# pfac-lib/PFAC

Hardware: AMD Instinct MI355X
Metric: input GB/s scanned (PFAC_matchFromDevice, bit-exact) (higher is better)
Workload: dtype u8

## Files before the change

### pfac_amd/csrc/scan_filter.hip

```cpp
#include "scan_common.h"

namespace {


#ifndef PFAC_ABLATE
#define PFAC_ABLATE 0
#endif
#ifndef PFAC_STATS
#define PFAC_STATS 0
#endif
constexpr int kGroupTiles = pfac::kChunkTiles;
constexpr int kGroupBytes = kGroupTiles * kTileBytes;
constexpr int kStageWords = (kGroupBytes + 48) / 4;
#ifndef PFAC_REFILL_MIN
#define PFAC_REFILL_MIN 16
#endif
#ifndef PFAC_REFILL_BATCH
#define PFAC_REFILL_BATCH 1
#endif
#ifndef PFAC_TIMING
#define PFAC_TIMING 0
#endif
#ifndef PFAC_LIST_CAP
#define PFAC_LIST_CAP 128
#endif
constexpr uint32_t kListCap = PFAC_LIST_CAP;
#ifndef PFAC_REDUCE_PARTS
#define PFAC_REDUCE_PARTS 32
#endif
#ifndef PFAC_APPEND_MIN
#define PFAC_APPEND_MIN 48
#endif
constexpr uint32_t kAppendMin = PFAC_APPEND_MIN;
#ifndef PFAC_MERGE_MIN
#define PFAC_MERGE_MIN 48
#endif
constexpr uint32_t kMergeMin = PFAC_MERGE_MIN;
static_assert(kMergeMin <= 64 && kMergeMin < kListCap, "left-over candidates are moved to the list's head one per lane");
#ifndef PFAC_PATCH_STAGED
#define PFAC_PATCH_STAGED 0
#endif
constexpr bool kStagedPatch = PFAC_PATCH_STAGED != 0;
constexpr uint32_t kReduceCap = 16;
#ifndef PFAC_FRONT_LOG2
#define PFAC_FRONT_LOG2 4
#endif

#ifndef PFAC_WRITERS
#define PFAC_WRITERS 3
#endif
#ifndef PFAC_SPAN_LOG2
#define PFAC_SPAN_LOG2 2
#endif
constexpr int kSpanLog2 = PFAC_SPAN_LOG2;
constexpr uint32_t kSpanChunks = 1u << kSpanLog2;
#ifndef PFAC_RUN_AHEAD
#define PFAC_RUN_AHEAD ((64u >> kSpanLog2) > 4u ? (64u >> kSpanLog2) : 4u)
#endif
constexpr uint32_t kRunAhead = PFAC_RUN_AHEAD;
constexpr uint32_t kRing = 2 * kRunAhead;
static_assert((kRing - kRunAhead) * kSpanChunks >= 2 * 16 + kSpanChunks, "ring slack covers the unresolved tickets of 16 waves");
constexpr uint32_t kEnd = 0xFFFFFFFFu;
struct Control {
    uint32_t popCount;
    uint32_t pubCount;
    uint32_t claimTurn;
    uint32_t endSpan;
    uint32_t ring[kRing];
};
constexpr int kControlWords = (sizeof(Control) / 4 + 3) / 4 * 4;

template <bool REDUCE, bool STAGE, int VETO = 0>
struct FilterLds {
    static constexpr bool kStageWalk = !REDUCE && STAGE;
    static constexpr int kWriters = REDUCE ? 0 : PFAC_WRITERS;
    static constexpr int kScanners = kWavesPerBlock - kWriters;
    static constexpr int kStageBufWords = kStageWalk ? (int)(kWalkStageBytes / 4) : kStageWords;
    static constexpr int kStageBufs = kStageWalk ? 2 : 1;
    enum Region { kQueue, kQueueB, kQueueC, kStage, kList, kPairs, kDense, kTrailing };
    static constexpr uint32_t kWaveWords[kTrailing] = {
        kQueueCap * (kStageWalk ? 1 : 4),
        kStageWalk ? 0 : kQueueCap * 2,
        (REDUCE || kStageWalk) ? 0 : kQueueCap * 4,
        (uint32_t)(kStageBufWords * kStageBufs),
        kListCap / 2,
        (REDUCE || kStagedPatch) ? 2 * kReduceCap : 0,
        REDUCE ? 0 : kDenseStage,
    };
    static constexpr uint32_t offsetWords(int r)
    {
        uint32_t w = kControlWords;
        for (int i = 0; i < r; i++) w += kScanners * kWaveWords[i];
        return w;
    }
    template <int R> static constexpr uint32_t kOffsetWords = offsetWords(R);
    static constexpr size_t kBufferBytes = 4 * (size_t)offsetWords(kTrailing);
    static constexpr size_t bytes(int log2BitsLad, int log2BitsF3, bool hasShort)
    {
        return (REDUCE ? pfac::reduceBitmapLdsBytes(log2BitsF3, hasShort) : pfac::filterBitmapLdsBytes(log2BitsLad, log2BitsF3, hasShort)) + kBufferBytes;
    }
};

__device__ __forceinline__ uint32_t ldsLoad(const uint32_t *p) { return __hip_atomic_load(p, __ATOMIC_RELAXED, __HIP_MEMORY_SCOPE_WORKGROUP); }
__device__ __forceinline__ void ldsStore(uint32_t *p, uint32_t v) { __hip_atomic_store(p, v, __ATOMIC_RELAXED, __HIP_MEMORY_SCOPE_WORKGROUP); }


__device__ __forceinline__ uint32_t waveMin(uint32_t v)
{
    auto step = [](uint32_t x, uint32_t y) { return y < x ? y : x; };
    v = step(v, (uint32_t)__builtin_amdgcn_update_dpp((int)v, (int)v, 0x111, 0xf, 0xf, false));
    v = step(v, (uint32_t)__builtin_amdgcn_update_dpp((int)v, (int)v, 0x112, 0xf, 0xf, false));
    v = step(v, (uint32_t)__builtin_amdgcn_update_dpp((int)v, (int)v, 0x114, 0xf, 0xf, false));
    v = step(v, (uint32_t)__builtin_amdgcn_update_dpp((int)v, (int)v, 0x118, 0xf, 0xf, false));
    v = step(v, (uint32_t)__builtin_amdgcn_update_dpp((int)v, (int)v, 0x142, 0xa, 0xf, false));
    v = step(v, (uint32_t)__builtin_amdgcn_update_dpp((int)v, (int)v, 0x143, 0xc, 0xf, false));
    return (uint32_t)__builtin_amdgcn_readlane((int)v, 63);
}

#ifndef PFAC_COMPILER_VGPRS
#define PFAC_COMPILER_VGPRS 59
#endif
constexpr int kCompilerVgprs = PFAC_COMPILER_VGPRS;

template <bool TEX, bool HAS_SHORT, bool REDUCE, int kWalkSets, bool STAGE, int VETO = 0>
__global__ __launch_bounds__(kBlockThreads, PFAC_MIN_WAVES_PER_SIMD) __attribute__((amdgpu_num_vgpr(kCompilerVgprs)))
void pfac_scan_filter(ScanArgs a)
{
    constexpr int kTilesPerIter = kGroupTiles;
    constexpr int kChunkBytes = kTilesPerIter * kTileBytes;
    using WCtx = ChainCtx<TEX>;
    constexpr uint32_t kEntry = (REDUCE || (!STAGE && VETO == 2)) ? kEntryBytes : kEntryBytesFull;
    constexpr bool kWideEntry = kEntry > kEntryBytes;
    using L = FilterLds<REDUCE, STAGE, VETO>;
    constexpr bool kStageWalk = L::kStageWalk;
    constexpr bool kVeto = !REDUCE && !STAGE && VETO != 0;
    constexpr bool kVetoG = kVeto && VETO == 2;
    constexpr uint32_t kListCapK = kVetoG ? 2u * kListCap : kListCap;
    static_assert(kListCapK * 2 <= kQueueCap * 16 || !kVetoG, "VETO = 2: the list lies in the place of the queue's bytes 20..35");
#ifndef PFAC_TAIL_ASK_MIN
#define PFAC_TAIL_ASK_MIN 8
#endif
    constexpr uint32_t kTailAskMin = PFAC_TAIL_ASK_MIN;
    using WLane = std::conditional_t<kStageWalk, StageLane<TEX>, ChainLane<TEX, kEntry, kVeto && VETO == 1>>;
    constexpr int kStageWordsK = L::kStageBufWords, kStageBufs = L::kStageBufs;
    constexpr int kHaloDwords = kStageWalk ? (int)(kWalkHalo / 4) : 12;
    extern __shared__ __attribute__((aligned(16))) unsigned char smem[];
    const int words3 = 1 << (a.log2Bits - 5), wordsLad = 1 << (a.log2BitsLad - 5), wordsF3 = 1 << (a.log2BitsF3 - 5);
    uint32_t *sGram3 = reinterpret_cast<uint32_t *>(smem);
    uint32_t *sLadder = sGram3 + kLadderLdsOffset / 4;
    uint32_t *sFinal3 = REDUCE ? sGram3 + (kGram1LdsOffset + kGram1LdsBytes) / 4 : sLadder + wordsLad;
    uint32_t *sShort = sFinal3 + wordsF3;
    constexpr int kWriters = L::kWriters, kScanners = L::kScanners;
    constexpr uint32_t kQCap = kQueueCap;
    Control *ctl = reinterpret_cast<Control *>(sShort + (HAS_SHORT ? pfac::kShortLdsBytes / 4 : 0));
    uint32_t *const sBuffers = reinterpret_cast<uint32_t *>(ctl);
    uint32_t *sQueueAll = sBuffers + L::template kOffsetWords<L::kQueue>;
    uint32_t *sQueueBAll = sBuffers + L::template kOffsetWords<L::kQueueB>, *sQueueCAll = sBuffers + L::template kOffsetWords<L::kQueueC>;
    uint32_t *sStageAll = sBuffers + L::template kOffsetWords<L::kStage>, *sListAll = sBuffers + L::template kOffsetWords<L::kList>;
    uint32_t *sReduceAll = sBuffers + L::template kOffsetWords<L::kPairs>, *sDenseAll = sBuffers + L::template kOffsetWords<L::kDense>;
    uint32_t *sHotAll = sBuffers + L::template kOffsetWords<L::kTrailing>;

    const int tid = threadIdx.x;
    if (__builtin_amdgcn_groupstaticsize() != 0) __builtin_trap();
    {
        auto copy16 = [&](uint32_t *dst, const void *src, int words) {
            const u32x4 *g = reinterpret_cast<const u32x4 *>(src);
            u32x4 *s = reinterpret_cast<u32x4 *>(dst);
            for (int i = tid; i < words / 4; i += kBlockThreads) s[i] = g[i];
        };
        if (REDUCE) {
            copy16(sGram3, a.prefix4, (int)(kPrefix4LdsBytes / 4));
            copy16(sGram3 + kGram1LdsOffset / 4, a.gram1, (int)(kGram1LdsBytes / 4));
        } else {
            copy16(sGram3, a.gram3, words3);
            copy16(sLadder, a.ladder, wordsLad);
        }
        copy16(sFinal3, a.final3, wordsF3);
        if (HAS_SHORT) copy16(sShort, a.shortBits, (int)(pfac::kShortLdsBytes / 4));
        if constexpr (kStageWalk) copy16(sHotAll, a.chainSlots, (int)a.hotSlots * 4);
        if constexpr (kVeto && !kVetoG) { if (a.tail != nullptr) copy16(sHotAll, a.tail, 3 << a.log2Tail); }
        if (tid < kControlWords) reinterpret_cast<uint32_t *>(ctl)[tid] = (tid == (int)(offsetof(Control, endSpan) / 4)) ? kEnd : 0u;
    }
    __syncthreads();

    const int lane = tid & 63;
    const int wave = __builtin_amdgcn_readfirstlane(tid >> 6);
    u32x4 *queue = reinterpret_cast<u32x4 *>(sQueueAll) + wave * kQCap;
    typedef uint32_t u32x2 __attribute__((ext_vector_type(2)));
    u32x2 *queueB = reinterpret_cast<u32x2 *>(sQueueBAll) + wave * kQCap;
    u32x4 *queueC = reinterpret_cast<u32x4 *>(sQueueCAll) + wave * kQCap;
    uint32_t *const stage0 = sStageAll + wave * (kStageWordsK * kStageBufs);
    uint32_t *stage = stage0;
    uint32_t *queue32 = sQueueAll + wave * kQCap;
    StageView view;
    view.addr[0] = (uint32_t)(reinterpret_cast<unsigned char *>(stage0) - smem);
    view.addr[1] = view.addr[0] + (uint32_t)kStageWordsK * 4u;
    view.base[0] = view.base[1] = 0;
    uint32_t cur = 0, qEnd[2] = {0, 0};
    bool modeStage = kStageWalk && __builtin_amdgcn_readfirstlane((int)a.work[pfac::kModeHintWord]) != 0;
    uint32_t deepRecent = 0, stageHold = modeStage ? 8u : 0u;
    uint16_t *list = kVetoG ? reinterpret_cast<uint16_t *>(sQueueCAll + wave * kQCap * 4) : reinterpret_cast<uint16_t *>(sListAll + wave * (kListCap / 2));
    const uint32_t n = (uint32_t)a.n;
    const Lds lds{sGram3, sLadder, sFinal3, sShort,
                  ((1u << ((uint32_t)a.log2Bits - 5u)) - 1u) << 2 , 32u - (uint32_t)a.log2BitsLad, 32u - (uint32_t)a.log2BitsF3};
#if PFAC_LADDER_BLOCKED
    uint32_t vLadMask;
    asm volatile("v_mov_b32 %0, %1" : "=v"(vLadMask) : "s"(((1u << ((uint32_t)a.log2BitsLad - 5u)) - 1u) << 2));
    auto ladWord = [&](uint32_t h) -> uint32_t {
        uint32_t addr;
        asm("v_and_b32_sdwa %0, %1, %2 dst_sel:DWORD dst_unused:UNUSED_PAD src0_sel:WORD_1 src1_sel:DWORD" : "=v"(addr) : "v"(h), "v"(vLadMask));
        return *reinterpret_cast<const __attribute__((address_space(3))) uint32_t *>(addr + kLadderLdsOffset);
    };
    auto ladStop = [](uint32_t w, uint32_t h) -> uint32_t { return (w >> ((h >> 3) & 31u)) & (w >> ((h >> 8) & 31u)); };
    auto ladGoOn = [](uint32_t w, uint32_t h) -> uint32_t { return w >> ((h >> 13) & 31u); };
    auto ladGoOn2 = [](uint32_t w, uint32_t h) -> uint32_t { return w >> (h & 31u); };
#else
    auto ladProbe = [&](uint32_t v) -> uint32_t {
        const uint32_t idx = v >> lds.shiftLad;
        return *reinterpret_cast<const __attribute__((address_space(3))) uint32_t *>(((idx >> 3) & ~3u) + kLadderLdsOffset) >> (idx & 31u);
    };
    auto ladWord = [](uint32_t h) -> uint32_t { return h; };
    auto ladStop = [&](uint32_t, uint32_t h) -> uint32_t { return ladProbe(h) & ladProbe(h * pfac::kLadMulS); };
    auto ladGoOn = [&](uint32_t, uint32_t h) -> uint32_t { return ladProbe(h * pfac::kLadMulG); };
    auto ladGoOn2 = [&](uint32_t, uint32_t h) -> uint32_t { return ladProbe(h * pfac::kLadMulG2); };
#endif
    WCtx wctx(a);
    if constexpr (kStageWalk) {
        wctx.hotAddr = (uint32_t)(reinterpret_cast<unsigned char *>(sHotAll) - smem);
        wctx.hotSlots = a.hotSlots;
    }
    WLane walk[kWalkSets];
    bool alive[kWalkSets];
#pragma unroll
    for (int s = 0; s < kWalkSets; s++) alive[s] = false;
    uint32_t qh = 0, qv = 0;
    constexpr uint32_t kMask = kQCap - 1;
    auto uni = [](uint32_t v) { return (uint32_t)__builtin_amdgcn_readfirstlane((int)v); };
    uint32_t stRounds = 0, stLaneSteps = 0, stStarts = 0, stHits = 0, stCand = 0;
#if PFAC_STATS
    uint32_t stFullRounds = 0, stSlotGathers = 0, stWinLoads = 0, stStartDead = 0;
#endif

    uint32_t *rPos = sReduceAll + wave * (2 * kReduceCap);
    uint32_t *rId = rPos + kReduceCap;
    uint32_t rn = 0;
    int pendMatch[kWalkSets];
    uint32_t pendPos[kWalkSets];
#pragma unroll
    for (int s = 0; s < kWalkSets; s++) { pendMatch[s] = 0; pendPos[s] = 0; }

    auto report = [&](bool ended, const WLane &w, int s) {
        if (ended & (w.match != 0)) {
            if (REDUCE || kStagedPatch) {
                pendMatch[s] = w.match;
                pendPos[s] = w.pos;
            } else {
#if defined(PFAC_EXP_PATCH_LOCAL)
                a.out[w.pos & 0xFFFFFu] = w.match;
#elif defined(PFAC_EXP_PATCH_NT)
                __builtin_nontemporal_store(w.match, &a.out[w.pos]);
#elif !defined(PFAC_EXP_NOSTORE)
                a.out[w.pos] = w.match;
#endif
            }
        }
    };
    auto flushStaged = [&]() {
        if (rn == 0) return;
        __builtin_amdgcn_fence(__ATOMIC_RELEASE, "wavefront");
        __builtin_amdgcn_fence(__ATOMIC_ACQUIRE, "wavefront");
        if (REDUCE) {
            unsigned int base = 0;
            if (lane == 0) base = atomicAdd(a.reduceCount, rn);
            base = (unsigned int)__builtin_amdgcn_readfirstlane((int)base);
            for (uint32_t i = lane; i < rn; i += 64) {
                a.out[base + i] = (int)rId[i];
                a.reducePos[base + i] = (int)(a.reduceBase + rPos[i]);
            }
        } else {
            if ((uint32_t)lane < rn) a.out[rPos[lane]] = (int)rId[lane];
        }
        rn = 0;
        __builtin_amdgcn_fence(__ATOMIC_RELEASE, "wavefront");
    };
    auto stagePending = [&]() {
        if (!REDUCE && !kStagedPatch) return;
#pragma unroll
        for (int s = 0; s < kWalkSets; s++) {
            const bool has = pendMatch[s] != 0;
            const uint64_t m = __ballot(has);
            if (m) {
                const uint32_t cnt = (uint32_t)__popcll(m);
                if (rn + cnt > kReduceCap) flushStaged();
                if (cnt > kReduceCap) {
                    if (REDUCE) {
                        unsigned int base = 0;
                        if (lane == 0) base = atomicAdd(a.reduceCount, cnt);
                        base = (unsigned int)__builtin_amdgcn_readfirstlane((int)base) + laneRankIn(m);
                        if (has) { a.out[base] = pendMatch[s]; a.reducePos[base] = (int)(a.reduceBase + pendPos[s]); pendMatch[s] = 0; }
                    } else if (has) {
                        a.out[pendPos[s]] = pendMatch[s];
                        pendMatch[s] = 0;
                    }
                } else {
                    const uint32_t at = rn + laneRankIn(m);
                    if (has) { rPos[at] = pendPos[s]; rId[at] = (uint32_t)pendMatch[s]; pendMatch[s] = 0; }
                    rn = uni(rn + cnt);
                }
            }
        }
    };
    constexpr bool kSpecKernel = WLane::kSpec;
    constexpr uint32_t kSpecOnScore = 16, kSpecOffRounds = 16;
#ifndef PFAC_SPEC_FORCE
#define PFAC_SPEC_FORCE -1
#endif
    int advBalance = 0;
    uint32_t chunkEvents = 0;
    bool specOn = PFAC_SPEC_FORCE == 1 || (PFAC_SPEC_FORCE < 0 && kStageWalk && modeStage);
    uint32_t specScore = 0, specIdle = 0;
    auto walkIssue = [&]() {
#pragma unroll
        for (int s = 0; s < kWalkSets; s++) {
            if (alive[s]) walk[s].issue(wctx, specOn);
            (void)view;
            stLaneSteps += (uint32_t)__popcll(__ballot(alive[s]));
        }
        stRounds++;
#if PFAC_STATS
#pragma unroll
        for (int s = 0; s < kWalkSets; s++) {
            stSlotGathers += (uint32_t)__popcll(__ballot(alive[s] && walk[s].needSlot));
            if constexpr (!kStageWalk) stWinLoads += (uint32_t)__popcll(__ballot(alive[s] && walk[s].needWin));
        }
#endif
    };
    auto walkConsume = [&]() {
#pragma unroll
        for (int s = 0; s < kWalkSets; s++) {
            bool cont = false;
            if (alive[s]) {
                if constexpr (kStageWalk) cont = walk[s].consume(wctx);
                else cont = walk[s].consume(wctx, specOn);
            }
            if (kSpecKernel && PFAC_SPEC_FORCE < 0) {
                if (!specOn) {
                    bool odd = walk[s].needExt;
                    if constexpr (kStageWalk) odd |= walk[s].ranOff;
                    if (__ballot(alive[s] & odd) != 0) {
                        chunkEvents += (uint32_t)__popcll(__ballot(alive[s] & odd));
                        if constexpr (kStageWalk) deepRecent += (uint32_t)__popcll(__ballot(alive[s] & walk[s].ranOff));
                        specScore += (uint32_t)__popcll(__ballot(alive[s] & walk[s].needExt));
                        if (specScore >= kSpecOnScore) { specOn = true; specScore = 0; specIdle = 0; }
                    }
                } else {
                    const uint32_t loaded = (uint32_t)__popcll(__ballot(alive[s] & walk[s].haveE)), used = (uint32_t)__popcll(__ballot(alive[s] & walk[s].usedE));
                    chunkEvents += used;
                    specIdle = (loaded < 8u || used * 4u < loaded) ? specIdle + 1u : 0u;
                    if (specIdle >= kSpecOffRounds) { specOn = false; specIdle = 0; }
                }
            }
            if constexpr (!REDUCE && !kStageWalk && !kSpecKernel) {
                const bool odd = walk[s].tookLong | walk[s].needWin;
                if (__ballot(alive[s] & odd) != 0) chunkEvents += (uint32_t)__popcll(__ballot(alive[s] & odd));
            }
            report(alive[s] & !cont, walk[s], s);
            alive[s] = cont;
        }
        stagePending();
    };
    constexpr uint32_t kRefillBatch = (uint32_t)PFAC_REFILL_BATCH < kQCap / 2 ? (uint32_t)PFAC_REFILL_BATCH : kQCap / 2;
    bool flushWalks = false;
#ifndef PFAC_WALK_GATE
#define PFAC_WALK_GATE 64
#endif
#ifndef PFAC_WALK_GATE_TRIPS
#define PFAC_WALK_GATE_TRIPS 6
#endif
    constexpr bool kWalkGated = !REDUCE && !kStageWalk && kWalkSets == 1 && PFAC_WALK_GATE > 0;
    constexpr uint32_t kWalkGate = PFAC_WALK_GATE, kWalkGateTrips = PFAC_WALK_GATE_TRIPS;
    uint32_t walkIdleTrips = 0;
    auto walkRefill = [&]() {
#pragma unroll
        for (int s = 0; s < kWalkSets; s++) {
            const uint64_t idle = __ballot(!alive[s]);
            const bool drainNow = kStageWalk && !modeStage && (uint32_t)__popcll(idle) >= qv - qh;
#ifndef PFAC_REFILL_MIN_STAGE
#define PFAC_REFILL_MIN_STAGE 6
#endif
            const uint32_t refillMin = (kStageWalk && modeStage) ? (uint32_t)PFAC_REFILL_MIN_STAGE : (uint32_t)PFAC_REFILL_MIN;
            if (((uint32_t)__popcll(idle) >= refillMin || drainNow) && qh != qv && (qv - qh >= kRefillBatch || flushWalks)) {
                __builtin_amdgcn_fence(__ATOMIC_ACQUIRE, "wavefront");
                const uint32_t rank = laneRankIn(idle);
                const bool take = !alive[s] & (rank < qv - qh);
                if (take) {
                    const uint32_t qi = (qh + rank) & kMask;
                    if constexpr (kStageWalk) {
#ifndef PFAC_LONG_JUMP
#define PFAC_LONG_JUMP 1
#endif
                        const bool longJump = PFAC_LONG_JUMP != 0 && specOn;
                        if (modeStage) walk[s].startStage(wctx, view, queue32[qi], HAS_SHORT ? sShort : nullptr, longJump);
                        else walk[s].startText(wctx, view, queue32[qi] & 0x7FFFFFFFu, view.addr[1] + ((uint32_t)s * 64u + (uint32_t)lane) * kWalkEntryBytes, HAS_SHORT ? sShort : nullptr, longJump);
                    } else {
                        const u32x2 eb = queueB[qi];
                        u32x4 ec = {0, 0, 0, 0};
                        if (kWideEntry) ec = queueC[qi];
                        walk[s].start(wctx, queue[qi], eb.x, eb.y, ec, HAS_SHORT ? sShort : nullptr);
                    }
                }
                alive[s] = alive[s] | take;
                const uint32_t idleLanes = (uint32_t)__popcll(idle);
                const uint32_t taken = idleLanes < qv - qh ? idleLanes : qv - qh;
                stStarts += taken;
                qh = uni(qh + taken);
            }
        }
    };
    auto anyAlive = [&]() {
        bool any = false;
#pragma unroll
        for (int s = 0; s < kWalkSets; s++) any |= alive[s];
        return __ballot(any) != 0;
    };

    const uint32_t numChunks = n / kChunkBytes;
    const uint32_t numPieces = kWriters ? (numChunks + kSpanChunks - 1) >> kSpanLog2 : numChunks;
    constexpr uint32_t kParts = REDUCE ? (uint32_t)PFAC_REDUCE_PARTS : (uint32_t)pfac::kWorkParts;
    const uint32_t parts = gridDim.x < kParts ? gridDim.x : kParts;
    const uint32_t part = blockIdx.x % parts;
    constexpr bool kFrontOn = PFAC_FRONT_LOG2 >= 0;
    constexpr uint32_t kFront = kFrontOn ? PFAC_FRONT_LOG2 : 0;
    const uint32_t partBegin = kFrontOn ? 0u : (uint32_t)((uint64_t)numPieces * part / parts);
    const uint32_t pieceEnd = kFrontOn ? numPieces : (uint32_t)((uint64_t)numPieces * (part + 1) / parts);
    auto pieceOf = [&](uint32_t v) {
        if (kFrontOn) return ((((v >> kFront) * parts + part) << kFront) | (v & ((1u << kFront) - 1u)));
        return partBegin + v;
    };
    unsigned int *const counter = a.work + part * 32;

    if (kWriters && wave >= kScanners) {
        const i32x4 zero = {0, 0, 0, 0};
#if PFAC_TIMING
        uint32_t wt[6] = {0, 0, 0, 0, 0, 0};
        uint64_t wLast = __builtin_readcyclecounter();
#define PFAC_WTICK(k) do { __builtin_amdgcn_sched_barrier(0); const uint64_t tNow = __builtin_readcyclecounter(); wt[k] += (uint32_t)(tNow - wLast); wLast = tNow; __builtin_amdgcn_sched_barrier(0); } while (0)
#else
#define PFAC_WTICK(k) do { } while (0)
#endif
        for (uint32_t k = (uint32_t)(wave - kScanners);; k += kWriters) {
#if PFAC_TIMING
            while (ldsLoad(&ctl->claimTurn) != k) __builtin_amdgcn_s_sleep(8);
            PFAC_WTICK(0);
#endif
            for (;;) {
                const uint32_t turn = ldsLoad(&ctl->claimTurn), pops = ldsLoad(&ctl->popCount);
                if (turn == k && k < (pops >> kSpanLog2) + kRunAhead) break;
                __builtin_amdgcn_s_sleep(8);
            }
            PFAC_WTICK(1);
            unsigned int v = 0;
            if (lane == 0) v = atomicAdd(counter, 1u);
            const uint32_t span = pieceOf(uni(v));
            PFAC_WTICK(2);
            ldsStore(&ctl->claimTurn, k + 1);
            if (span >= pieceEnd) {
                if (lane == 0) atomicMin(&ctl->endSpan, k);
                break;
            }
            const uint32_t c0 = span << kSpanLog2;
            const uint32_t cN = c0 + kSpanChunks < numChunks ? c0 + kSpanChunks : numChunks;
            i32x4 *o4 = reinterpret_cast<i32x4 *>(a.out + (size_t)c0 * kChunkBytes);
            const uint32_t stores = (cN - c0) * (kChunkBytes * 4 / 1024);
            for (uint32_t i = 0; i < stores; i++) __builtin_nontemporal_store(zero, &o4[i * 64 + lane]);
            PFAC_WTICK(3);
            asm volatile("s_waitcnt vmcnt(0)" ::: "memory");
            PFAC_WTICK(4);
            while (ldsLoad(&ctl->pubCount) != k) __builtin_amdgcn_s_sleep(2);
            ldsStore(&ctl->ring[k & (kRing - 1)], span);
            __builtin_amdgcn_fence(__ATOMIC_RELEASE, "workgroup");
            ldsStore(&ctl->pubCount, k + 1);
            PFAC_WTICK(5);
        }
#if PFAC_TIMING
        if (lane == 0)
            for (int k = 0; k < 6; k++) atomicAdd(reinterpret_cast<unsigned long long *>(a.work + pfac::kStatsWord) + 20 + k, (unsigned long long)wt[k]);
#endif
    } else {
    if (a.endsIn != nullptr) {
// ... 291 lines not shown
                }
                stagedBase = chunk * kChunkBytes;
                if constexpr (kStageWalk) { if (cur) view.base[1] = stagedBase; else view.base[0] = stagedBase; }
                freshChunk = true;
                PFAC_TICK(3);
                const uint32_t next = resolve(nextTicket);
                PFAC_TICK(6);
                prefetchChunk(next != kEnd ? next : chunk);
                chunk = next;
                nextTicket = uni(afterNext);
#if PFAC_ABLATE == 1
                ablateSink |= hits;
                hits = 0;
#endif
            }
        }
        if ((listAt == listEnd || (!REDUCE && listEnd - listAt < kMergeMin)) && __ballot(hits != 0) != 0) {
            const uint32_t carry = listEnd - listAt;
            if (carry != 0 && listAt != 0) {
                const uint32_t code = (uint32_t)lane < carry ? listCode(listAt) : 0u;
                if ((uint32_t)lane < carry) list[lane] = (uint16_t)code;
                __builtin_amdgcn_fence(__ATOMIC_RELEASE, "wavefront");
                __builtin_amdgcn_fence(__ATOMIC_ACQUIRE, "wavefront");
            }
            const uint32_t cnt = (uint32_t)__builtin_popcount(hits);
            const uint32_t incl = waveInclusiveScan(cnt);
            const uint32_t total = (uint32_t)__builtin_amdgcn_readlane((int)incl, 63);
            uint32_t idx = carry + incl - cnt;
            PFAC_TICK(9);
            const bool dense = !REDUCE && freshChunk && total > kDenseHits && a.denseList != nullptr;
            if (dense) {
                if (lane == 0) sDense[nDense] = stagedBase / (uint32_t)kChunkBytes;
                nDense++;
                if (nDense == kDenseStage) flushDense();
                hits = 0;
            }
            freshChunk = false;
            while (hits != 0 && idx < kListCapK) {
                list[idx] = (uint16_t)(((uint32_t)lane << 5) | (uint32_t)__builtin_ctz(hits));
                idx++;
                hits &= hits - 1;
            }
            PFAC_TICK(10);
            const uint32_t listed = dense ? 0u : (total < kListCapK - carry ? total : kListCapK - carry);
#ifndef PFAC_COUNT_STALLS
            stHits += listed;
#endif
            __builtin_amdgcn_fence(__ATOMIC_RELEASE, "wavefront");
            __builtin_amdgcn_fence(__ATOMIC_ACQUIRE, "wavefront");
            PFAC_TICK(4);
            uint32_t kept = carry;
            for (uint32_t base = 0; base < listed; base += 64u) {
                const bool act = base + (uint32_t)lane < listed;
                const uint32_t code = act ? listCode(carry + base) : 0u;
                const uint32_t o = ((code & 0x10u) << 6) | ((code >> 1) & 0x3F0u) | (code & 0xFu);
                const uint32_t at = o >> 2, sh = o & 3u;
                const uint32_t x = __builtin_amdgcn_alignbyte(stage[at + 1], stage[at], sh);
                const uint32_t h = REDUCE ? x * pfac::kLadMul0 : (x * pfac::kLadMul0) ^ a.ladderSalt;
                uint32_t sHit, gHit;
                if (REDUCE) {
                    auto probe4 = [&](uint32_t v) -> uint32_t {
                        const uint32_t idx = v >> (32 - pfac::kPrefix4Log2);
                        return *reinterpret_cast<const __attribute__((address_space(3))) uint32_t *>((idx >> 3) & ~3u) >> (idx & 31u);
                    };
                    sHit = probe4(h) & probe4(h * pfac::kLadMulS) & 1u;
                    gHit = 0;
                } else {
                    const uint32_t w = ladWord(h);
                    sHit = ladStop(w, h) & 1u;
                    gHit = ladGoOn(w, h) & ladGoOn2(w, h) & 1u;
                }
                uint32_t decided = sHit | (testBit(sFinal3, (uint32_t)__umul24(x, pfac::kFinal3Mul) >> lds.shiftF3) &
                                           testBit(sFinal3, (uint32_t)__umul24(x, pfac::kFinal3Mul2) >> lds.shiftF3));
                if (HAS_SHORT) decided |= testBit(sShort, x & 0xFFFFu);
                const bool keep = act && (decided | gHit) != 0;
                const uint64_t keepMask = __ballot(keep);
                if (keep) list[kept + laneRankIn(keepMask)] = (uint16_t)(code | (decided << 15));
                kept = uni(kept + (uint32_t)__popcll(keepMask));
            }
            listAt = 0;
            listEnd = kept;
            stCand += kept - carry;
            __builtin_amdgcn_fence(__ATOMIC_RELEASE, "wavefront");
            __builtin_amdgcn_fence(__ATOMIC_ACQUIRE, "wavefront");
            PFAC_TICK(11);
        }
        for (;;) {
            const uint32_t left = listEnd - listAt;
            const uint32_t want = left < 64u ? left : 64u;
            const uint32_t room = kQCap - (qv - qh) - pendCount;
            const uint32_t take = room < want ? room : want;
            if (left == 0 || (take != want && take < kAppendMin)) break;
            if (!REDUCE && left < kMergeMin && __ballot(hits != 0) != 0) break;
            const bool act = (uint32_t)lane < take;
            const uint32_t code = act ? listCode(listAt) : 0u;
            const uint32_t o = ((code & 0x10u) << 6) | ((code >> 1) & 0x3F0u) | (code & 0xFu);
            const uint32_t at = o >> 2, sh = o & 3u;
            const uint32_t e0 = stage[at], e1 = stage[at + 1], e2 = stage[at + 2], e3 = stage[at + 3], e4 = stage[at + 4], e5 = stage[at + 5];
            const uint32_t x0 = __builtin_amdgcn_alignbyte(e1, e0, sh), x1 = __builtin_amdgcn_alignbyte(e2, e1, sh), x2 = __builtin_amdgcn_alignbyte(e3, e2, sh),
                           x3 = __builtin_amdgcn_alignbyte(e4, e3, sh), x4 = __builtin_amdgcn_alignbyte(e5, e4, sh);
            uint32_t walk = act ? (code >> 15) & 1u : 0u;
            uint32_t und = act ? walk ^ 1u : 0u;
            const uint32_t und0 = (uint32_t)__popcll(__ballot(und != 0));
            const bool skipLadder = !REDUCE && ladderSkip != 0;
            const bool deepLadder = a.ladderLast > pfac::kLadderLast;
            uint32_t stopHash = 0;
            (void)stopHash;
            if (skipLadder) { ladderSkip--; walk |= und; und = 0; }
            if (!REDUCE && __ballot(und != 0) != 0) {
                uint32_t hl[pfac::kLadderLevels];
                hl[0] = (x0 * pfac::kLadMul0) ^ a.ladderSalt;
#pragma unroll
                for (int lv = 1; lv < pfac::kLadderLevels; lv++) {
                    const uint32_t xw = lv <= 2 ? x1 : lv <= 4 ? x2 : lv <= 6 ? x3 : x4;
                    hl[lv] = (hl[lv - 1] ^ ((lv & 1) ? (xw & 0xFFFFu) : (xw >> 16))) * pfac::kLadMul;
                }
                uint32_t skipping = 0;
                bool straightToLast = false;
                if (a.skipCount != 0) {
                    for (int k = 0; k < a.skipCount; k++) skipping |= hl[1] == a.skipTags[k] ? 1u : 0u;
                    skipping &= und;
                }
#pragma unroll
                for (int lv = 1; lv < pfac::kLadderLevels; lv++) {
                    if (lv == 5 && __ballot(und != 0) == 0) break;
                    if (lv >= 2 && lv <= 4 && a.skipCount != 0 && !straightToLast) straightToLast = __ballot((und & ~skipping) != 0) == 0;
                    if (lv >= 2 && lv < pfac::kLadderLevels - 1 && straightToLast) continue;
                    const uint32_t act = (lv >= 2 && lv < pfac::kLadderLevels - 1) ? (und & ~skipping) : und;
                    const uint32_t h = hl[lv];
                    const uint32_t w = ladWord(h);
                    const uint32_t sHit = ladStop(w, h);
                    if constexpr (kVeto) stopHash = (act & sHit) ? h : stopHash;
                    walk |= act & sHit;
                    if (lv == pfac::kLadderLevels - 1 && !deepLadder) und = 0;
                    else und &= ~act | (ladGoOn(w, h) & ~sHit);
                }
                if constexpr (kVeto) {
                    if (deepLadder && __ballot(und != 0) != 0) {
                        uint32_t h = hl[pfac::kLadderLevels - 1];
                        const uint32_t staged = (uint32_t)kChunkBytes + 4u * (uint32_t)kHaloDwords;
                        for (uint32_t dd = (uint32_t)pfac::kLadderLast; dd < (uint32_t)a.ladderLast && __ballot(und != 0) != 0; dd += 8u) {
                            const bool any = und != 0u && o + dd + 12u <= staged;
                            walk |= any ? 0u : und;
                            und = any ? und : 0u;
                            const uint32_t b = any ? o + dd : 0u;
                            const uint32_t w0 = stage[b >> 2], w1 = stage[(b >> 2) + 1u], w2 = stage[(b >> 2) + 2u];
                            const uint32_t lo = __builtin_amdgcn_alignbyte(w1, w0, b & 3u), hi = __builtin_amdgcn_alignbyte(w2, w1, b & 3u);
                            uint32_t hk[4], wk[4];
#pragma unroll
                            for (int k = 0; k < 4; k++) {
                                const uint32_t piece = ((k < 2 ? lo : hi) >> (16 * (k & 1))) & 0xFFFFu;
                                h = (h ^ piece) * pfac::kLadMul;
                                hk[k] = h;
                            }
#pragma unroll
                            for (int k = 0; k < 4; k++) wk[k] = ladWord(hk[k]);
#pragma unroll
                            for (int k = 0; k < 4; k++) {
                                const bool lvl = dd + 2u * (uint32_t)k < (uint32_t)a.ladderLast;
                                const uint32_t sHit = ladStop(wk[k], hk[k]);
                                stopHash = (lvl && (und & sHit & 1u)) ? hk[k] : stopHash;
                                walk |= lvl ? (und & sHit) : 0u;
                                und = lvl ? (und & ladGoOn(wk[k], hk[k]) & ~sHit) : und;
                            }
                        }
                    }
                }
                walk |= und;
                if constexpr (kVeto) {
                    const bool ask = a.tail != nullptr && stopHash != 0u && (walk & 1u) != 0u;
                    if constexpr (kVetoG) {
                        if (!pendAny && (uint32_t)__popcll(__ballot(ask)) >= kTailAskMin) {
                            pendCode = ask ? (0x80000000u | o) : 0u;
                            pendHash = stopHash;
                            pendAny = true;
                            pendCount = (uint32_t)__popcll(__ballot(ask));
                            walk = ask ? 0u : walk;
                        }
                    } else if (__ballot(ask) != 0) {
                        const uint32_t *sTail = sHotAll;
                        const uint32_t tshift = 32u - (uint32_t)a.log2Tail;
                        const uint32_t s1 = ((uint32_t)(stopHash * pfac::kTailMul) >> tshift) * 3u, s2 = ((uint32_t)(stopHash * pfac::kTailMul2) >> tshift) * 3u;
                        const uint32_t t1 = sTail[s1], h1 = sTail[s1 + 1], i1 = sTail[s1 + 2], t2 = sTail[s2], h2 = sTail[s2 + 1], i2 = sTail[s2 + 2];
                        const bool m1 = i1 != 0u && t1 == stopHash, m2 = i2 != 0u && t2 == stopHash;
                        const uint32_t want = m1 ? h1 : h2, info = m1 ? i1 : (m2 ? i2 : 0u);
                        const uint32_t nb = info & 0xFFu, from = o + (info >> 8);
                        const bool chk = ask && info != 0u && from + nb + 4u <= (uint32_t)kChunkBytes + 4u * (uint32_t)kHaloDwords;
                        const bool vetoed = chk && tailRun(stopHash, chk, from, nb) != want;
                        if (vetoed) walk = 0u;
                        chunkEvents += (uint32_t)__popcll(__ballot(vetoed));
                    }
                }
            }
            if (REDUCE) walk |= und;
            if (!REDUCE && !skipLadder && und0 >= 16u) {
                const uint32_t walked = (uint32_t)__popcll(__ballot(walk != 0)) - (take - und0);
                ladderIdle = (und0 - walked) * 8u < und0 ? ladderIdle + 1u : 0u;
                if (ladderIdle >= 4u) { ladderIdle = 0; ladderSkip = 28; }
            }
#if PFAC_ABLATE >= 3
            walk = (((o * 2654435761u) >> 28) < (PFAC_ABLATE - 2) * 4u) ? walk : 0u;
#endif
            const bool keep = walk != 0;
            const uint64_t keepMask = __ballot(keep);
            if (keep) {
                const uint32_t qi = (qv + laneRankIn(keepMask)) & kMask;
                if constexpr (kStageWalk) {
                    queue32[qi] = (cur << 31) | o;
                } else {
                const u32x4 entry = {stagedBase + o, x0, x1, x2};
                const u32x2 entryB = {x3, x4};
                queue[qi] = entry;
                queueB[qi] = entryB;
                if (kWideEntry) {
                    const uint32_t e6 = stage[at + 6], e7 = stage[at + 7], e8 = stage[at + 8], e9 = stage[at + 9];
                    const u32x4 entryC = {__builtin_amdgcn_alignbyte(e6, e5, sh), __builtin_amdgcn_alignbyte(e7, e6, sh),
                                          __builtin_amdgcn_alignbyte(e8, e7, sh), __builtin_amdgcn_alignbyte(e9, e8, sh)};
                    queueC[qi] = entryC;
                }
                }
            }
            qv = uni(qv + (uint32_t)__popcll(keepMask));
            listAt = uni(listAt + take);
        }
        if constexpr (kVetoG) {
            if (pendAny && (pendCode >> 31) != 0u)
                pendE = reinterpret_cast<const u32x4 *>(a.tail)[(uint32_t)(pendHash * pfac::kTailMul) >> (32u - (uint32_t)a.log2Tail)];
        }
        __builtin_amdgcn_fence(__ATOMIC_RELEASE, "wavefront");
        PFAC_TICK(5);
#if PFAC_ABLATE == 2
        qh = qv;
#endif
    }
#if PFAC_ABLATE == 1
    if (ablateSink == 0x12345u) a.out[0] = 1;
#endif
    if (REDUCE || kStagedPatch) flushStaged();
    if (!REDUCE && a.denseList != nullptr) flushDense();
#if PFAC_TIMING
    if (lane == 0)
        for (int k = 0; k < 12; k++) atomicAdd(reinterpret_cast<unsigned long long *>(a.work + pfac::kStatsWord) + 8 + k, (unsigned long long)tm[k]);
#endif
    }

    __syncthreads();
    if (tid < 8) sGram3[tid] = 0;
    __syncthreads();
    if (lane == 0) {
        atomicAdd(&sGram3[0], stRounds); atomicAdd(&sGram3[1], stLaneSteps);
        atomicAdd(&sGram3[2], stStarts); atomicAdd(&sGram3[3], stHits); atomicAdd(&sGram3[4], stCand);
        if (!REDUCE && advBalance > 0 && !(kWriters && wave >= kScanners)) atomicAdd(&sGram3[5], 1u);
    }
    __syncthreads();
    if (tid < 4) atomicAdd(reinterpret_cast<unsigned long long *>(a.work + pfac::kStatsWord) + tid, (unsigned long long)sGram3[tid]);
    if (tid == 5) atomicAdd(reinterpret_cast<unsigned long long *>(a.work + pfac::kStatsWord) + 5, (unsigned long long)sGram3[4]);
    if (!REDUCE && tid == 6 && sGram3[5] != 0) atomicAdd(a.work + pfac::kModeVotesWord, sGram3[5]);
    if (wave == 0) {
        __threadfence();
        unsigned int before = 0;
        if (lane == 0) before = atomicAdd(a.work + pfac::kDoneWord, 1u);
        before = (unsigned int)__builtin_amdgcn_readfirstlane((int)before);
        if (before == gridDim.x - 1u) {
            __threadfence();
            unsigned long long *acc = reinterpret_cast<unsigned long long *>(a.work + pfac::kStatsWord);
            unsigned long long *published = reinterpret_cast<unsigned long long *>(a.work + pfac::kStatsPublishedWord);
            if (lane < 32) atomicExch(a.work + lane * 32, 0u);
            if (lane < pfac::kStatsCount) published[lane] = lane == 4 ? (unsigned long long)a.n : atomicExch(acc + lane, 0ull);
            if (lane == pfac::kStatsCount) {
                const unsigned int denseChunks = REDUCE ? 0u : atomicAdd(a.work + a.denseWord, 0u);
                published[lane] = (unsigned long long)denseChunks;
                if (!REDUCE && a.hostHint != nullptr) __hip_atomic_store(a.hostHint + 1, denseChunks * 2u > numChunks ? 1u : 0u, __ATOMIC_RELAXED, __HIP_MEMORY_SCOPE_SYSTEM);
            }
            if (lane == pfac::kStatsCount + 1) published[lane] = (unsigned long long)kWalkSets;
            if (lane == pfac::kStatsCount + 2) {
                const unsigned int votes = !REDUCE ? atomicExch(a.work + pfac::kModeVotesWord, 0u) : 0u;
                published[lane] = (unsigned long long)votes | ((unsigned long long)(kStageWalk ? 1u : 0u) << 32) | ((unsigned long long)(kVeto ? (kVetoG ? 2u : 1u) : 0u) << 33);
                if (!REDUCE) {
                    const unsigned int hint = votes * 2u >= gridDim.x * (unsigned int)kScanners ? 1u : 0u;
                    atomicExch(a.work + pfac::kModeHintWord, hint);
                    if (a.hostHint != nullptr) __hip_atomic_store(a.hostHint, hint, __ATOMIC_RELAXED, __HIP_MEMORY_SCOPE_SYSTEM);
                }
            }
            if (lane == 32) atomicExch(a.work + a.denseWordOther, 0u);
            if (lane == 33) atomicExch(a.work + pfac::kDoneWord, 0u);
        }
    }
#if PFAC_STATS
    if (lane == 0 && (blockIdx.x % 32) == 0 && wave == 0)
        printf("STATS block %d wave0 fullRounds %u slotGathers %u winLoads %u startDead %u\n", (int)blockIdx.x, stFullRounds, stSlotGathers, stWinLoads, stStartDead);
#endif
}


using LdsWindow = FilterLds<false, false>;
using LdsStage = FilterLds<false, true>;
using LdsReduce = FilterLds<true, false>;
static_assert(pfac::kFilterLdsBudget + (LdsWindow::kBufferBytes > LdsStage::kBufferBytes ? LdsWindow::kBufferBytes : LdsStage::kBufferBytes) <= kLdsPerCu,
              "prefilter bitmaps + scanning waves' buffers must fit the CU's LDS");
static_assert(LdsReduce::bytes(0, 13, true) <= kLdsPerCu, "compacted-output kernel: gram1 + prefix4 + final3 + short bitmap + scanning waves' buffers must fit the CU's LDS");
static_assert(pfac::kFilterLdsBudget + FilterLds<false, false, 1>::kBufferBytes <= kLdsPerCu, "a tail table that the pattern compiler keeps in LDS must find room there");
constexpr bool kShippedShape = kWavesPerBlock == 16 && PFAC_WRITERS == 3 && kQueueCap == 64 && kListCap == 128 && kRing == 32 && !kStagedPatch;
template <class LDS> constexpr bool ldsTotalsAre(size_t plain, size_t withShort) { return !kShippedShape || (LDS::bytes(19, 13, false) == plain && LDS::bytes(19, 13, true) == withShort); }
static_assert(ldsTotalsAre<LdsWindow>(163744, 171936), "window walker");
static_assert(ldsTotalsAre<LdsStage>(163120, 171312), "stage walker, before its hot slots");
static_assert(ldsTotalsAre<FilterLds<false, false, 2>>(163744, 171936), "VETO = 2: the window walker's, with the list in queueC's place");
static_assert(ldsTotalsAre<LdsReduce>(147344, 155536), "compacted output");

size_t filterLdsBytes(const PFAC_context *c, bool reduce, bool stage)
{
    const pfac::Filter &f = c->filter;
    auto total = [&](auto lds) { return lds.bytes(f.log2BitsLad, f.log2BitsF3, f.hasShort); };
    return reduce ? total(LdsReduce{}) : stage ? total(LdsStage{}) : total(LdsWindow{});
}

size_t vetoLdsBytes(const PFAC_context *c, const ScanArgs &a)
{
    if (a.tail == nullptr || a.log2Tail < 2 || c->filter.tail.empty()) return 0;
    const size_t bytes = size_t(12) << a.log2Tail;
    return filterLdsBytes(c, false, false) + bytes <= kLdsPerCu ? bytes : 0;
}

template <bool TEX, bool HAS_SHORT, bool REDUCE, bool STAGE, int VETO = 0>
hipError_t launchFilter(const PFAC_context *c, const ScanArgs &a0)
{
    auto kernel = pfac_scan_filter<TEX, HAS_SHORT, REDUCE, REDUCE ? PFAC_WALK_SETS : PFAC_WALK_SETS_FULL, STAGE, VETO>;
    static ShapeCache cache;
    size_t lds = filterLdsBytes(c, REDUCE, STAGE) + (VETO == 1 ? vetoLdsBytes(c, a0) : 0);
    int dev = -1;
    hipError_t de = hipGetDevice(&dev);
    if (de != hipSuccess) return de;
    if (lds > kLdsPerCu || dev < 0 || dev >= kMaxDevices) return hipErrorInvalidValue;
    ScanArgs a = a0;
    a.hotSlots = 0;
    if (!REDUCE && STAGE) {
#ifndef PFAC_FILTER_HOT
#define PFAC_FILTER_HOT 1
#endif
        size_t hot = PFAC_FILTER_HOT ? (kLdsPerCu - lds) / sizeof(pfac::ChainSlot) : 0;
        const size_t top = (size_t)a.rootRow + (size_t)pfac::kCharSet;
        if (hot > top) hot = top;
        if (hot < 1024) hot = 0;
        a.hotSlots = (uint32_t)hot;
        lds += hot * sizeof(pfac::ChainSlot);
    }
    int perCU;
    {
        std::lock_guard<std::mutex> g(cache.lock);
        if (cache.perCU[dev] == 0) {
            hipError_t e = hipFuncSetAttribute(reinterpret_cast<const void *>(kernel),
                                               hipFuncAttributeMaxDynamicSharedMemorySize, (int)kLdsPerCu);
            if (e != hipSuccess) return e;
            int n = 0;
            e = hipOccupancyMaxActiveBlocksPerMultiprocessor(&n, kernel, kBlockThreads, kLdsPerCu);
            if (e != hipSuccess) return e;
            cache.perCU[dev] = n < 1 ? 1 : n;
        }
        perCU = cache.perCU[dev];
    }
    const size_t numChunks = a.n / kChunkBytesHost;
    constexpr size_t scanners = FilterLds<REDUCE, STAGE, VETO>::kScanners;
    size_t blocks = (numChunks + scanners - 1) / scanners;
    const size_t resident = (size_t)(c->multiProcessorCount > 0 ? c->multiProcessorCount : 256) * perCU;
    if (blocks > resident) blocks = resident;
    hipError_t e = hipSuccess;
    if (PFAC_TIMING || c->countersDirty) {
        e = hipMemsetAsync(c->tables.workCounters.get(), 0, pfac::kWorkCounterWords * sizeof(unsigned int), 0);
        if (e != hipSuccess) return e;
        c->countersDirty = false;
    }
    const bool timed = c->kernelTiming && c->evTime[0] && c->evTime[1];
    if (timed) (void)hipEventRecord(static_cast<hipEvent_t>(c->evTime[0]), 0);
    hipLaunchKernelGGL(kernel, dim3((unsigned)blocks), dim3(kBlockThreads), lds, 0, a);
    e = hipGetLastError();
    if (e != hipSuccess) c->countersDirty = true;
    if (timed) c->evTimeRecorded = hipEventRecord(static_cast<hipEvent_t>(c->evTime[1]), 0) == hipSuccess;
#if PFAC_TIMING
    {
        unsigned long long t[18];
        (void)hipDeviceSynchronize();
        (void)hipMemcpy(t, c->tables.workCounters.get() + pfac::kStatsWord + 16, sizeof(t), hipMemcpyDeviceToHost);
        double sum = 0;
        for (int k = 0; k < 12; k++) sum += (double)t[k];
        static const char *names[12] = {"consume", "refill", "issue", "level1+stage", "list-fences", "ladder+append", "resolve(wait for writers)+prefetch issue", "loop/pop/other",
                                        "wait for loads (top of trip)", "popcount+scan", "emit-loop", "level-4 test"};
        fprintf(stderr, "PFAC_TIMING blocks %zu scanners %zu:", blocks, scanners);
        for (int k = 0; k < 12; k++) fprintf(stderr, "  %s %.1f%% (%.0f cyc/wave)", names[k], 100.0 * t[k] / sum, (double)t[k] / (blocks * scanners));
        if (!REDUCE && PFAC_WRITERS) {
            static const char *wnames[6] = {"wait for the other writer's claim", "wait for run-ahead room (scanners)", "device claim (atomic)", "issue zero stores",
                                            "wait until the zeros are in L2", "publish in order"};
            double wsum = 0;
            for (int k = 0; k < 6; k++) wsum += (double)t[12 + k];
            fprintf(stderr, "\nPFAC_TIMING writers %d per block:", (int)PFAC_WRITERS);
            for (int k = 0; k < 6; k++) fprintf(stderr, "  %s %.1f%% (%.0f cyc/wave)", wnames[k], 100.0 * t[12 + k] / wsum, (double)t[12 + k] / (blocks * PFAC_WRITERS));
        }
        fprintf(stderr, "\n");
    }
#endif
    return e;
}

#ifndef PFAC_QUICK
#define PFAC_QUICK 0
#endif

template <bool REDUCE, bool STAGE, int VETO>
hipError_t launchInstance(const PFAC_context *c, const ScanArgs &a, bool tex)
{
    const bool hasShort = c->filter.hasShort;
    if (tex) return hasShort ? launchFilter<true, true, REDUCE, STAGE, VETO>(c, a) : launchFilter<true, false, REDUCE, STAGE, VETO>(c, a);
    if constexpr (PFAC_QUICK) return hipErrorNotSupported;
    else return hasShort ? launchFilter<false, true, REDUCE, STAGE, VETO>(c, a) : launchFilter<false, false, REDUCE, STAGE, VETO>(c, a);
}

template <bool REDUCE>
hipError_t launchChained(const PFAC_context *c, const ScanArgs &a, bool tex)
{
    bool stage = false;
    int veto = 0;
    if (!REDUCE) {
#ifndef PFAC_VETO
#define PFAC_VETO 1
#endif
        const bool nearMisses = c->h_modeHint != nullptr && *static_cast<volatile const unsigned int *>(c->h_modeHint) != 0;
        if (PFAC_VETO && c->walker != PFACX_WALKER_STAGE) {
            if (vetoLdsBytes(c, a) != 0) veto = 1;
            else if (a.tail != nullptr && !c->filter.tailG.empty() && (c->walker == PFACX_WALKER_VETO || (c->walker == PFACX_WALKER_AUTO && nearMisses))) veto = 2;
        }
        stage = c->walker == PFACX_WALKER_STAGE || (veto == 0 && c->walker == PFACX_WALKER_AUTO && nearMisses);
    }
    if constexpr (PFAC_QUICK && REDUCE) return hipErrorNotSupported;
    else {
        if (veto == 2) return launchInstance<false, false, 2>(c, a, tex);
        if (veto) return launchInstance<false, false, 1>(c, a, tex);
        if (stage) return launchInstance<false, true, 0>(c, a, tex);
        return launchInstance<REDUCE, false, 0>(c, a, tex);
    }
}

}

namespace pfacmod {
hipError_t launchFilterKernel(const PFAC_context *c, const ScanArgs &a, bool tex, bool reduce)
{
    return reduce ? launchChained<true>(c, a, tex) : launchChained<false>(c, a, tex);
}
}
```

Baseline: 1240.

## Let writer waves skip the LDS table fill and batch scanner prefetch loads

Replaces the block-wide table copy into LDS plus __syncthreads with a fill done only by the scanner waves. Loads are batched eight deep across a flattened list of pieces, and scanners then wait on an LDS counter (fillDone) rather than a block barrier. Writer waves skip the fill and go straight into their loop, so their startup overlaps the fill. This adds a spin-wait and a control word (16 more bytes of LDS), and shrinks the set of threads doing the copy.

```diff
diff --git a/pfac_amd/csrc/scan_filter.hip b/pfac_amd/csrc/scan_filter.hip
--- a/pfac_amd/csrc/scan_filter.hip
+++ b/pfac_amd/csrc/scan_filter.hip
@@ -67,6 +67,7 @@
     uint32_t claimTurn;
     uint32_t endSpan;
     uint32_t ring[kRing];
+    uint32_t fillDone;
 };
 constexpr int kControlWords = (sizeof(Control) / 4 + 3) / 4 * 4;
 
@@ -161,30 +162,71 @@
     uint32_t *sHotAll = sBuffers + L::template kOffsetWords<L::kTrailing>;
 
     const int tid = threadIdx.x;
+    const int lane = tid & 63;
+    const int wave = __builtin_amdgcn_readfirstlane(tid >> 6);
     if (__builtin_amdgcn_groupstaticsize() != 0) __builtin_trap();
-    {
-        auto copy16 = [&](uint32_t *dst, const void *src, int words) {
-            const u32x4 *g = reinterpret_cast<const u32x4 *>(src);
-            u32x4 *s = reinterpret_cast<u32x4 *>(dst);
-            for (int i = tid; i < words / 4; i += kBlockThreads) s[i] = g[i];
+    constexpr bool kEarlyWriters = kWriters > 0;
+    if (tid < kControlWords) reinterpret_cast<uint32_t *>(ctl)[tid] = (tid == (int)(offsetof(Control, endSpan) / 4)) ? kEnd : 0u;
+    if constexpr (kEarlyWriters) __syncthreads();
+    if (!kEarlyWriters || wave < kScanners) {
+        constexpr uint32_t kFillThreads = kEarlyWriters ? (uint32_t)kScanners * 64u : (uint32_t)kBlockThreads;
+        constexpr int kFillBatch = 8, kFillPieces = 6;
+        const void *src[kFillPieces];
+        uint32_t dstAddr[kFillPieces], begin[kFillPieces + 1];
+        int pieces = 0;
+        begin[0] = 0;
+        auto piece = [&](const uint32_t *dst, const void *from, uint32_t words) {
+            src[pieces] = from;
+            dstAddr[pieces] = (uint32_t)(reinterpret_cast<const unsigned char *>(dst) - smem);
+            begin[pieces + 1] = begin[pieces] + words / 4u;
+            pieces++;
         };
         if (REDUCE) {
-            copy16(sGram3, a.prefix4, (int)(kPrefix4LdsBytes / 4));
-            copy16(sGram3 + kGram1LdsOffset / 4, a.gram1, (int)(kGram1LdsBytes / 4));
+            piece(sGram3, a.prefix4, (uint32_t)(kPrefix4LdsBytes / 4));
+            piece(sGram3 + kGram1LdsOffset / 4, a.gram1, (uint32_t)(kGram1LdsBytes / 4));
         } else {
-            copy16(sGram3, a.gram3, words3);
-            copy16(sLadder, a.ladder, wordsLad);
-        }
-        copy16(sFinal3, a.final3, wordsF3);
-        if (HAS_SHORT) copy16(sShort, a.shortBits, (int)(pfac::kShortLdsBytes / 4));
-        if constexpr (kStageWalk) copy16(sHotAll, a.chainSlots, (int)a.hotSlots * 4);
-        if constexpr (kVeto && !kVetoG) { if (a.tail != nullptr) copy16(sHotAll, a.tail, 3 << a.log2Tail); }
-        if (tid < kControlWords) reinterpret_cast<uint32_t *>(ctl)[tid] = (tid == (int)(offsetof(Control, endSpan) / 4)) ? kEnd : 0u;
-    }
-    __syncthreads();
-
-    const int lane = tid & 63;
-    const int wave = __builtin_amdgcn_readfirstlane(tid >> 6);
+            piece(sGram3, a.gram3, (uint32_t)words3);
+            piece(sLadder, a.ladder, (uint32_t)wordsLad);
+        }
+        piece(sFinal3, a.final3, (uint32_t)wordsF3);
+        piece(sShort, a.shortBits, HAS_SHORT ? (uint32_t)(pfac::kShortLdsBytes / 4) : 0u);
+        piece(sHotAll, a.chainSlots, kStageWalk ? a.hotSlots * 4u : 0u);
+        piece(sHotAll, a.tail, (kVeto && !kVetoG && a.tail != nullptr) ? 3u << a.log2Tail : 0u);
+        static_assert(kFillPieces == 6, "six pieces are listed");
+        const uint32_t total = begin[kFillPieces];
+        for (uint32_t base = (uint32_t)tid; base < total; base += kFillThreads * (uint32_t)kFillBatch) {
+            u32x4 r[kFillBatch];
+#pragma unroll
+            for (int j = 0; j < kFillBatch; j++) {
+                const uint32_t at = base + (uint32_t)j * kFillThreads, i = at < total ? at : total - 1u;
+                const void *from = src[0];
+                uint32_t off = i;
+#pragma unroll
+                for (int p = 1; p < kFillPieces; p++)
+                    if (i >= begin[p]) { from = src[p]; off = i - begin[p]; }
+                r[j] = reinterpret_cast<const u32x4 *>(from)[off];
+            }
+            asm volatile("" ::: "memory");
+#pragma unroll
+            for (int j = 0; j < kFillBatch; j++) {
+                const uint32_t i = base + (uint32_t)j * kFillThreads;
+                uint32_t to = dstAddr[0] + i * 16u;
+#pragma unroll
+                for (int p = 1; p < kFillPieces; p++)
+                    if (i >= begin[p]) to = dstAddr[p] + (i - begin[p]) * 16u;
+                if (i < total) *reinterpret_cast<u32x4 *>(smem + to) = r[j];
+            }
+        }
+        if constexpr (kEarlyWriters) {
+            __builtin_amdgcn_fence(__ATOMIC_RELEASE, "workgroup");
+            asm volatile("s_waitcnt lgkmcnt(0)" ::: "memory");
+            if (lane == 0) __hip_atomic_fetch_add(&ctl->fillDone, 1u, __ATOMIC_RELAXED, __HIP_MEMORY_SCOPE_WORKGROUP);
+            while (ldsLoad(&ctl->fillDone) != (uint32_t)kScanners) __builtin_amdgcn_s_sleep(1);
+            __builtin_amdgcn_fence(__ATOMIC_ACQUIRE, "workgroup");
+        }
+    }
+    if constexpr (!kEarlyWriters) __syncthreads();
+
     u32x4 *queue = reinterpret_cast<u32x4 *>(sQueueAll) + wave * kQCap;
     typedef uint32_t u32x2 __attribute__((ext_vector_type(2)));
     u32x2 *queueB = reinterpret_cast<u32x2 *>(sQueueBAll) + wave * kQCap;
@@ -1082,10 +1124,11 @@
 static_assert(pfac::kFilterLdsBudget + FilterLds<false, false, 1>::kBufferBytes <= kLdsPerCu, "a tail table that the pattern compiler keeps in LDS must find room there");
 constexpr bool kShippedShape = kWavesPerBlock == 16 && PFAC_WRITERS == 3 && kQueueCap == 64 && kListCap == 128 && kRing == 32 && !kStagedPatch;
 template <class LDS> constexpr bool ldsTotalsAre(size_t plain, size_t withShort) { return !kShippedShape || (LDS::bytes(19, 13, false) == plain && LDS::bytes(19, 13, true) == withShort); }
-static_assert(ldsTotalsAre<LdsWindow>(163744, 171936), "window walker");
-static_assert(ldsTotalsAre<LdsStage>(163120, 171312), "stage walker, before its hot slots");
-static_assert(ldsTotalsAre<FilterLds<false, false, 2>>(163744, 171936), "VETO = 2: the window walker's, with the list in queueC's place");
-static_assert(ldsTotalsAre<LdsReduce>(147344, 155536), "compacted output");
+static_assert(sizeof(Control) == 4 * (5 + kRing) && kControlWords * 4 >= (int)sizeof(Control) && kControlWords % 4 == 0, "the control block: five counters and the ring, padded to 16 bytes");
+static_assert(ldsTotalsAre<LdsWindow>(163760, 171952), "window walker");
+static_assert(ldsTotalsAre<LdsStage>(163136, 171328), "stage walker, before its hot slots");
+static_assert(ldsTotalsAre<FilterLds<false, false, 2>>(163760, 171952), "VETO = 2: the window walker's, with the list in queueC's place");
+static_assert(ldsTotalsAre<LdsReduce>(147360, 155552), "compacted output");
 
 size_t filterLdsBytes(const PFAC_context *c, bool reduce, bool stage)
 {
```

Result: no change. 1242, median of 6 (+0.2%).
